# jakovdev/SequenceAligner

Measured on AMD Instinct MI355X. Metric: pair-alignments/sec, higher is better.
Workload: dtype u16x2; 1 GPU; cfg2: 10000 protein seqs x U[80,120], nw blosum62 {'gap_pen': 4}, all-vs-all packed triangular; pairs=49995000, cells=501594494441, parallelism=pair-range x1

## Files before the change

### sequencealigner_amd/csrc/sa_context.hip

```cpp
#include <algorithm>
#include <cmath>
#include <cstdio>
#include <cstdlib>
#include <cstring>

#include "sa_ctx.h"

bool sa_device_ready(int device)
{
	int count = 0;
	hipError_t err = hipGetDeviceCount(&count);
	if (err != hipSuccess || count <= 0) {
		sa_set_error("No HIP devices available (%s); libseqalign_hip has no CPU fallback",
			     err == hipSuccess ? "device count is 0" : hipGetErrorString(err));
		return false;
	}
	if (device < 0 || device >= count) {
		sa_set_error("HIP device %d out of range (%d visible)", device, count);
		return false;
	}
	SA_HIP_CHECK(hipSetDevice(device), return false);
	return true;
}

// ... 90 lines not shown
	in.min_len = ctx->min_len;
	in.method = ctx->sc.method;
	in.gap_ext = ctx->sc.gap_ext;
	in.sys_ok = ctx->sys_ok;
	in.pk_kmax = ctx->pk_kmax;
	in.pk16_kmax = ctx->pk16_kmax;
	in.pk16_f16_kmax = ctx->pk16_f16_kmax;
	in.pk_chunk_cap = ctx->pk_chunk_cap;
	in.pk_q = ctx->pk_q;
	in.pk_floor = ctx->pk_floor;
	in.pk_gain = ctx->pk_gain;
	in.pk_slack = ctx->pk_slack;
	in.persistent_wgs = ctx->persistent_wgs;
	in.env_chunk = ctx->env.chunk;
	in.no_sort = ctx->env.no_sort;
	return in;
}

namespace {
struct CtxDeleter {
	void operator()(sa_ctx *c) const { sa_ctx_destroy(c); }
};
}

static sa_ctx *ctx_create_impl(int device, struct sa_input in, const struct sa_scoring *sc)
{
	if (!sc) {
		sa_set_error("sa_ctx_create: null scoring");
		return nullptr;
	}
// ... 271 lines not shown
```

### sequencealigner_amd/csrc/sa_env.cpp

```cpp
#include "sa_env.h"

#include <algorithm>
#include <cstdlib>

static bool flag(const char *name) { return getenv(name) != nullptr; }
static int number(const char *name, int fallback, int lo, int hi)
{
	const char *v = getenv(name);
	if (!v || !*v)
		return fallback;
	return std::max(lo, std::min(hi, atoi(v)));
}

SaEnv sa_env_read()
{
	SaEnv e;
	e.force_generic = flag("SA_HIP_FORCE_GENERIC");
	e.no_pk = flag("SA_HIP_NO_PK");
	e.no_pk16 = flag("SA_HIP_NO_PK16");
	e.no_sort = flag("SA_HIP_NO_SORT");
	e.chunk = number("SA_HIP_CHUNK", 0, 1, 32);
	e.stagger = number("SA_HIP_STAGGER", 0, 0, 64);
	e.no_pin = flag("SA_HIP_NO_PIN");
	e.no_direct = flag("SA_HIP_NO_DIRECT");
	e.no_shells = flag("SA_HIP_NO_SHELLS");
	e.devices = number("SA_HIP_DEVICES", 0, 0, 1024);
	e.split = number("SA_HIP_SPLIT", 0, 0, 1024);
	e.gather = getenv("SA_HIP_GATHER") ? (atoi(getenv("SA_HIP_GATHER")) != 0) : -1;
	e.tiles_split = number("SA_HIP_TILES_SPLIT", 0, 0, 64);
	e.trace_batch_bytes = getenv("SA_HIP_TRACE_BATCH_BYTES") ? std::max(0LL, atoll(getenv("SA_HIP_TRACE_BATCH_BYTES"))) : 0LL;
	e.verbose = flag("SA_HIP_VERBOSE");
	e.stamps = flag("SA_HIP_STAMPS");
	e.stamps_dump = getenv("SA_HIP_STAMPS_DUMP");
	e.ztrace = flag("SA_HIP_ZTRACE");
	return e;
// ... 2 lines not shown
```

### sequencealigner_amd/csrc/sa_env.h

```cpp
#ifndef SA_ENV_H
#define SA_ENV_H

struct SaEnv {
	bool force_generic = false;
	bool no_pk = false;
	bool no_pk16 = false;
	bool no_sort = false;
	int chunk = 0;
	int stagger = 0;
	bool no_pin = false;
	bool no_direct = false;
	bool no_shells = false;
	int devices = 0;
	int split = 0;
	int gather = -1;
	int tiles_split = 0;
	long long trace_batch_bytes = 0;
	bool verbose = false;
	bool stamps = false;
	const char *stamps_dump = nullptr;
	bool ztrace = false;
};

SaEnv sa_env_read();
// ... 3 lines not shown
```

### sequencealigner_amd/csrc/sa_internal.h

```cpp
#ifndef SA_INTERNAL_H
#define SA_INTERNAL_H

#include <hip/hip_runtime.h>
#include <cstdint>
#include <cstdarg>
#include <string>
#include <vector>


#include "sa_shapes.h"

#define SA_HIP_CHECK(call, onfail)                                                  \
	if (hipError_t err__ = (call); err__ != hipSuccess) {                       \
		sa_set_error("%s failed: %s", #call, hipGetErrorString(err__));      \
		onfail;                                                              \
	} else                                                                      \
		(void)0

struct SaSeqStore {
	const uint8_t *codes;
	const struct sa_meta *meta;
	int32_t num;
};

// ... 19 lines not shown
	int64_t start, end;
	int32_t *out;
	int32_t out16;
	int32_t pconst;
	int32_t q;
	int32_t gap_g, gap_o, gap_e;
	int32_t delta;
	int32_t chunk;
	int32_t *long_scratch;
	int64_t long_stride;
	int32_t pk_base;
	const SaArranged *lvp;
	int32_t npart;
	int32_t out_nt;
	int32_t pk_f16;
	const int32_t *tlist;
	const int64_t *dense_off;
	int32_t *host_out;
	int32_t nlocal;
	const SaPkClassArgs *pkc;
	const uint32_t *ulist;
	int32_t tile_pair;
	int32_t npkc;
	unsigned *counter;
	int32_t rotate_prio;
	int32_t stagger;
	int32_t stamp_u;
	unsigned long long *stamps;
};

// ... 29 lines not shown
```

### sequencealigner_amd/csrc/sa_launch.hip

```cpp
#include <algorithm>
#include <cstdio>
#include <cstring>

#include "sa_ctx.h"


static void plan_free_device(sa_ctx::Plan &pl)
{
	for (auto &c : pl.dc) {
		(void)hipFree(c.d_jlist);
		(void)hipFree(c.d_tprefix);
		(void)hipFree(c.d_tlist);
		(void)hipFree(c.d_doff);
	}
	(void)hipFree(pl.d_segs);
	for (auto &b : pl.db) {
		(void)hipFree(b.d_args);
		(void)hipFree(b.d_ulist);
	}
	pl.dc.clear();
	pl.db.clear();
	pl.d_segs = nullptr;
}

// ... 248 lines not shown
	if (!ctx->timing)
		return true;
	SA_HIP_CHECK(hipEventRecord(e1, s), return false);
	ctx->events.push_back(sa_ctx::Timed{ name, e0, e1, pairs, cells });
	return true;
}

static Launch pk_launch(const sa_ctx *ctx, const sa_ctx::Plan &pl, size_t bi, int rk, bool share, unsigned *counters, const SaSysArgs &common)
{
	const SaHostBundle &b = pl.h.bundles[bi];
	Launch L;
	L.is_pk = true;
	L.g = b.g;
	L.klo = b.klo;
	L.f16 = b.f16;
	L.lds = (unsigned)sa_pk_lds_bytes(ctx->sc.method, b.g, b.kmax);
	SaSysArgs &a = L.a = common;
	a.pconst = ctx->pk_pconst;
	a.q = ctx->sc.method == SA_METHOD_SW ? 0 : ctx->pk_q;
	a.out_nt = ctx->out_is_host && !share ? 1 : 0;
	a.pk_f16 = b.f16;
	a.chunk = pl.h.chunk_pk;
	a.stagger = ctx->env.stagger;
	a.rotate_prio = ctx->sc.method != SA_METHOD_NW;
	a.pkc = pl.db[bi].d_args;
	a.ulist = pl.db[bi].d_ulist + b.ufirst[(size_t)rk];
	a.npkc = (int32_t)b.cls.size();
	a.nlocal = L.ntiles = b.nlocal[(size_t)rk];
	a.counter = counters + 2 * (SA_PK_CLASS0 + (int)bi);
	L.pairs = b.pairs[(size_t)rk];
	L.cells = b.cells[(size_t)rk];
	L.nstamp = (size_t)L.ntiles;
	L.stamp_words = 7 * L.nstamp;
	L.wgs = (int)std::min<int64_t>(ctx->persistent_wgs / 32 * (ctx->leave_room ? 3 : 4), L.ntiles);
	int klo_seen = b.kmax;
	for (int ci : b.cls)
		klo_seen = std::min(klo_seen, sa_pk_decode(pl.h.classes[(size_t)ci].cls).k);
	snprintf(L.name, sizeof(L.name), "sa_k_systolic_pk_bundle<%s,%d,%d,%s>[K%d-%d]", METHOD_TAG[ctx->sc.method], b.g, b.klo,
		 b.f16 ? "true" : "false", klo_seen, b.kmax);
	return L;
}

static bool long_scratch_ready(sa_ctx *ctx)
{
	if (ctx->d_long_scratch)
		return true;
	ctx->long_stride = 2 * (16 * ((int64_t)ctx->max_len + 1) + 64);
	const int64_t budget_ints = ((int64_t)4 << 30) / 4;
	const int64_t wpb = SA_SYS_WPB(64, true);
	ctx->long_wgs = (int)std::max<int64_t>(16, std::min<int64_t>(ctx->persistent_wgs / 4, budget_ints / (ctx->long_stride * wpb)));
	SA_HIP_CHECK(hipMalloc(&ctx->d_long_scratch, sizeof(int32_t) * (size_t)(ctx->long_stride * ctx->long_wgs * wpb)), return false);
	return true;
}

// ... 331 lines not shown
```

### sequencealigner_amd/csrc/sa_plan.cpp

```cpp
#include "sa_plan.h"
#include "sa_guard.h"

#include <algorithm>
#include <cmath>
#include <cstdlib>

int32_t sa_column_of(int64_t p)
{
	int64_t j = (int64_t)((1.0 + std::sqrt(1.0 + 8.0 * (double)p)) * 0.5);
	while (j * (j - 1) / 2 > p)
		--j;
	while ((j + 1) * j / 2 <= p)
		++j;
	return (int32_t)j;
}

SaPairPlan::SaPairPlan(const sa_meta *m, int32_t n) : num(n), pairs((int64_t)n * (n - 1) / 2), meta(m)
{
	len_prefix.assign((size_t)n + 1, 0);
	cell_prefix.assign((size_t)n + 1, 0);
	for (int32_t k = 0; k < n; k++) {
		len_prefix[(size_t)k + 1] = len_prefix[(size_t)k] + m[k].len;
		cell_prefix[(size_t)k + 1] = cell_prefix[(size_t)k] + (int64_t)m[k].len * len_prefix[(size_t)k];
	}
// ... 37 lines not shown
}

bool sa_arranged_exists(int32_t num, const SaArrKey &key)
{
	const int64_t wave_rows = (int64_t)key.ng * key.ch;
	return key.block > 0 && wave_rows > 0 && key.block % (wave_rows * SA_PK_WPB) == 0 && key.block <= num;
}

int sa_pk_arranged_keys(const SaPlanInputs &in, int pk_g, int pk_k, int32_t chunk_pk, bool host_out, SaArrKey (&lv)[SA_PK_SORT_LEVELS])
{
	for (auto &x : lv)
		x = SaArrKey{};
	if (in.no_sort || chunk_pk <= 0)
		return 0;
	const int ng = 64 / pk_g;
	const int32_t rows = sa_pk_wpb(in.method, pk_g, pk_k) * ng * chunk_pk;
	int nl = 0;
	for (int l = 0; l < SA_PK_SORT_LEVELS; l++) {
		const int32_t block = SA_PK_SORT_ROWS >> l;
		if (host_out || rows >= SA_PK_ROWS_OWN_BLOCK || block <= rows || block % rows != 0)
			continue;
		const SaArrKey key{ ng, chunk_pk, block };
		if (sa_arranged_exists(in.num, key))
			lv[nl++] = key;
	}
	if (nl < SA_PK_SORT_LEVELS) {
		const SaArrKey key{ ng, chunk_pk, rows };
		if (sa_arranged_exists(in.num, key))
			lv[nl++] = key;
	}
	return nl;
// ... 54 lines not shown
	std::vector<std::vector<int32_t>> jl((size_t)SA_PLAN_NCLASSES), tp((size_t)SA_PLAN_NCLASSES);
	std::vector<int64_t> cpairs((size_t)SA_PLAN_NCLASSES, 0), ccells((size_t)SA_PLAN_NCLASSES, 0);
	std::vector<std::vector<std::pair<int32_t, int32_t>>> rows_of((size_t)SA_PLAN_NCLASSES);
	std::vector<int64_t> lenpre((size_t)num + 1, 0);
	for (int32_t k = 0; k < num; k++)
		lenpre[(size_t)k + 1] = lenpre[(size_t)k] + in.meta[k].len;
	{
		const int64_t want_tiles = (int64_t)in.persistent_wgs * 6;
		const int64_t mine = world > 1 ? count / world : count;
		int32_t chunk = SA_SYS_CHUNK;
		while (chunk > 8 && mine / (4 * chunk) < want_tiles)
			chunk >>= 1;
		if (in.env_chunk)
			chunk = in.env_chunk;
		plan.chunk = chunk;
		const int64_t want_pk = (int64_t)in.persistent_wgs * 5 / 8;
		int32_t cpk = SA_SYS_CHUNK;
		while (cpk > 4 && mine / ((int64_t)2 * SA_PK_WPB * 8 * cpk) < want_pk)
			cpk >>= 1;
		if (in.env_chunk)
			cpk = in.env_chunk;
		cpk = std::min(cpk, in.pk_chunk_cap);
		plan.chunk_pk = cpk;
		constexpr int TWO_SIZES_BELOW = 16, SMALL_TILE_DIV = 4, SMALL_PAIRS_FRAC = 5;
		const int64_t slots = (int64_t)in.persistent_wgs / 8;
		if (!in.env_chunk && mine / ((int64_t)2 * SA_PK_WPB * 8 * cpk) < (int64_t)TWO_SIZES_BELOW * slots) {
			int32_t big = SA_SYS_CHUNK;
			while (big > 16 && 2 * mine / ((int64_t)2 * SA_PK_WPB * 8 * big) < 5 * slots)
				big >>= 1;
			big = std::min(std::max(big, cpk), in.pk_chunk_cap);
			if (big >= 16) {
				plan.chunk_pk = big;
				plan.chunk_pk_small = std::max(4, big / SMALL_TILE_DIV);
				const int64_t jlo = sa_column_of(start), jhi = sa_column_of(end - 1) + 1;
				int64_t lo = jlo, hi = jhi;
				while (lo < hi) {
					const int64_t mid = (lo + hi) / 2;
					if (mid * (mid - 1) / 2 - start >= count / SMALL_PAIRS_FRAC)
						hi = mid;
					else
						lo = mid + 1;
				}
				plan.j_small = (int32_t)lo;
// ... 33 lines not shown
			sa_set_error("%s", TOO_LARGE);
			return false;
		}
		jl[(size_t)cls].push_back(j);
		tp[(size_t)cls].push_back(tp[(size_t)cls].back() + (int32_t)tiles);
		cpairs[(size_t)cls] += ib - ia;
		ccells[(size_t)cls] += (int64_t)n * (lenpre[(size_t)ib] - lenpre[(size_t)ia]);
	}
	std::vector<int32_t> nparts((size_t)SA_PLAN_NCLASSES, 0);
	std::vector<std::vector<int32_t>> part_rows((size_t)SA_PLAN_NCLASSES);
	for (int cls = SA_PK_CLASS0; cls < SA_PLAN_NCLASSES; cls++) {
		const auto &rw = rows_of[(size_t)cls];
		if (rw.empty())
			continue;
		const SaPkCls pc = sa_pk_decode(cls);
		const int64_t rows = (int64_t)sa_pk_wpb(in.method, pc.g, pc.k) * (64 / pc.g) * (pc.small ? plan.chunk_pk_small : plan.chunk_pk);
		tp[(size_t)cls].push_back(0);
		std::vector<std::pair<int32_t, int32_t>> parts;
		for (size_t c = 0; c < rw.size(); c += 2) {
			const auto &a = rw[c], &b = rw[c + 1 < rw.size() ? c + 1 : c];
			const int64_t span = std::max(a.second, b.second) - std::min(a.first, b.first);
			const int64_t tiles = span / rows;
			if ((int64_t)tp[(size_t)cls].back() + tiles + (int64_t)parts.size() + 1 > ((int64_t)1 << SA_PK_UTILE_BITS)) {
				sa_set_error("%s", TOO_LARGE);
				return false;
			}
			tp[(size_t)cls].push_back(tp[(size_t)cls].back() + (int32_t)tiles);
			if (span % rows)
				parts.emplace_back((int32_t)(span % rows), (int32_t)(c / 2));
		}
		std::stable_sort(parts.begin(), parts.end(), [](const auto &x, const auto &y) { return x.first > y.first; });
// ... 42 lines not shown
		for (size_t ci = 0; ci < plan.classes.size(); ci++) {
			auto &cl = plan.classes[ci];
			const int cls = cl.cls;
			const bool is_pk = cls >= SA_PK_CLASS0;
			const int pk_g = is_pk ? sa_pk_decode(cls).g : 8;
			const int G = is_pk ? pk_g : cls == SA_SYS_CLASS_LONG ? 64 : SA_SYS_CLASSES[cls].G;
			const int K = is_pk ? sa_pk_decode(cls).k : cls == SA_SYS_CLASS_LONG ? 16 : SA_SYS_CLASSES[cls].K;
			const int64_t weight = (int64_t)(K + 6) * (G / 8);
			const auto &J = cl.jlist;
			const auto &T = cl.tprefix;
			std::vector<Geo> tiles((size_t)cl.ntiles);
			if (is_pk) {
				SaArrKey lv[SA_PK_SORT_LEVELS];
				sa_pk_arranged_keys(in, pk_g, K, cl.chunk, share_host, lv);
				const int32_t lvrows[SA_PK_SORT_LEVELS] = { lv[0].block, lv[1].block, lv[2].block, lv[3].block };
				const int32_t rows = sa_pk_wpb(in.method, pk_g, K) * (64 / pk_g) * cl.chunk;
				const auto &rw = rows_of[(size_t)cls];
				const int32_t npairs = (cl.ncols + 1) / 2, nfull = T[(size_t)npairs];
				for (int32_t t = 0; t < cl.ntiles; t++) {
					int32_t lo;
					if (t < nfull)
						lo = (int32_t)(std::upper_bound(T.begin(), T.begin() + npairs + 1, t) - T.begin()) - 1;
					else
						lo = T[(size_t)(npairs + 1 + (t - nfull))];
					const size_t c0 = (size_t)2 * (size_t)lo, c1 = c0 + 1 < rw.size() ? c0 + 1 : c0;
					Geo &g = tiles[(size_t)t];
					g.dup = c1 == c0;
					g.j[0] = J[c0], g.j[1] = J[c1];
					g.ia[0] = rw[c0].first, g.ib[0] = rw[c0].second;
					g.ia[1] = rw[c1].first, g.ib[1] = rw[c1].second;
					const int32_t ra = std::min(g.ia[0], g.ia[1]), rb = std::max(g.ib[0], g.ib[1]);
// ... 102 lines not shown
		}
	}
	const int nranks = std::max(world, 1);
	std::vector<int> order;
	for (size_t ci = 0; ci < plan.classes.size(); ci++)
		if (plan.classes[ci].cls >= SA_PK_CLASS0)
			order.push_back((int)ci);
	std::sort(order.begin(), order.end(), [&](int x, int y) { return plan.classes[(size_t)x].cls > plan.classes[(size_t)y].cls; });
	std::stable_partition(order.begin(), order.end(), [&](int x) { return !sa_pk_decode(plan.classes[(size_t)x].cls).small; });
	for (int ci : order) {
		const auto &cl = plan.classes[(size_t)ci];
		const int g = sa_pk_decode(cl.cls).g;
		const int k = sa_pk_decode(cl.cls).k;
		const int klo = sa_pk_bundle_klo(g, k);
		const int f16 = g == 8 || k <= in.pk16_f16_kmax ? 1 : 0;
		SaHostBundle *b = nullptr;
		for (auto &x : plan.bundles)
			if (x.g == g && x.klo == klo && x.f16 == f16)
				b = &x;
		if (!b) {
			plan.bundles.emplace_back();
			b = &plan.bundles.back();
			b->g = g, b->klo = klo, b->f16 = f16, b->kmax = k;
		}
		b->kmax = std::max(b->kmax, k);
		b->cls.push_back(ci);
	}
	for (auto &b : plan.bundles) {
		b.args.resize(b.cls.size());
		for (size_t x = 0; x < b.cls.size(); x++) {
			const auto &cl = plan.classes[(size_t)b.cls[x]];
			const int k = sa_pk_decode(cl.cls).k;
			SaHostPkArgs &a = b.args[x];
			sa_pk_arranged_keys(in, b.g, k, cl.chunk, share_host, a.lv);
			a.cls_index = b.cls[x];
			a.chunk = cl.chunk;
			a.ncols = cl.ncols;
			a.npart = cl.npart;
// ... 7 lines not shown
		b.pairs.assign((size_t)nranks, 0);
		b.cells.assign((size_t)nranks, 0);
		struct Part {
			int64_t work;
			uint32_t code, pair;
		};
		std::vector<Part> parts;
		for (int r = 0; r < nranks; r++) {
			parts.clear();
			for (size_t x = 0; x < b.cls.size(); x++) {
				const auto &cl = plan.classes[(size_t)b.cls[x]];
				const int32_t nfull = cl.ntiles - cl.npart;
				const auto &T = cl.tprefix;
				const int32_t npairs = (cl.ncols + 1) / 2;
				const bool small = sa_pk_decode(cl.cls).small;
				const int64_t full_rows = (int64_t)sa_pk_wpb(in.method, b.g, sa_pk_decode(cl.cls).k) * (64 / b.g) * cl.chunk;
				int32_t pair_of_full = 0;
				for (int32_t t = 0; t < cl.ntiles; t++) {
					uint32_t pair;
					if (t < nfull) {
						while (pair_of_full + 1 < npairs && T[(size_t)pair_of_full + 1] <= t)
							pair_of_full++;
						pair = (uint32_t)pair_of_full;
					} else {
						pair = (uint32_t)T[(size_t)(npairs + 1 + (t - nfull))];
					}
					if (world >= 1 && cl.owner[(size_t)t] != r)
						continue;
					const uint32_t code = ((uint32_t)x << SA_PK_UTILE_BITS) | (uint32_t)t;
					if (t < nfull && !small) {
						ul.push_back(code);
// ... 63 lines not shown
```

### sequencealigner_amd/csrc/sa_plan.h

```cpp
#ifndef SA_PLAN_H
#define SA_PLAN_H

#include <cstdint>
#include <string>
#include <utility>
#include <vector>

#include "sa_shapes.h"

int32_t sa_column_of(int64_t p);
inline int64_t sa_tri(int64_t j) { return j * (j - 1) / 2; }

struct SaPairPlan {
	int32_t num = 0;
	int64_t pairs = 0;
	const sa_meta *meta = nullptr;
	std::vector<int64_t> len_prefix;
	std::vector<int64_t> cell_prefix;
	SaPairPlan(const sa_meta *m, int32_t n);
	int64_t cells_before(int64_t p) const;
};

struct SaArrKey {
	int ng = 0, ch = 0;
// ... 4 lines not shown
inline int sa_pk_live(int32_t min_len, int g) { return 1 + (g - 1) / ((min_len > 1 ? min_len : 1) + 1); }

struct SaPlanInputs {
	int32_t num = 0;
	const sa_meta *meta = nullptr;
	int32_t min_len = 1;
	int method = 0;
	int32_t gap_ext = 0;
	bool sys_ok = false;
	int pk_kmax = 0, pk16_kmax = 0, pk16_f16_kmax = 0, pk_chunk_cap = SA_SYS_CHUNK;
	int32_t pk_q = 0, pk_floor = 0;
	int64_t pk_gain = 0, pk_slack = 0;
	int persistent_wgs = 256 * 32;
	int env_chunk = 0;
	bool no_sort = false;
};

struct SaKernelLimits {
	bool sys_ok = false;
	int32_t sys_pconst = 0, sys_q = 0;
	int64_t sys_gain = 0, sys_slack = 0;
	int pk_kmax = 0, pk16_kmax = 0, pk16_f16_kmax = 0, pk_chunk_cap = SA_SYS_CHUNK;
	int32_t pk_pconst = 0, pk_q = 0, pk_floor = 0;
	int64_t pk_gain = 0, pk_slack = 0, pk_extra = 0;
};
SaKernelLimits sa_kernel_limits(const sa_scoring &sc, int32_t max_len, int32_t min_len, bool force_generic, bool no_pk, bool no_pk16);

int32_t sa_pk_delta(const SaPlanInputs &in, int g, int k);
int32_t sa_pk_base(const SaPlanInputs &in, int g, int k);

// ... 26 lines not shown
struct SaHostSeg {
	int64_t src, dst;
	int32_t count, pos0, ia, ib, flags;
	int map_kind;
	SaArrKey key;
};

struct SaHostPkArgs {
	int cls_index = 0;
	int32_t ncols = 0, npart = 0, k = 0, delta = 0, pk_base = 0, chunk = 0;
	SaArrKey lv[SA_PK_SORT_LEVELS];
};

struct SaHostBundle {
	int g = 8, klo = 1, f16 = 1, kmax = 1;
	std::vector<int> cls;
	std::vector<SaHostPkArgs> args;
	std::vector<uint32_t> ulist;
	std::vector<int64_t> ufirst;
	std::vector<int32_t> nlocal;
	std::vector<int64_t> pairs, cells;
};

struct SaGenericShare {
	int64_t start, count, doff;
};

struct SaHostPlan {
	int64_t start = -1, count = -1;
	int32_t chunk = SA_SYS_CHUNK;
// ... 17 lines not shown
```

### sequencealigner_amd/csrc/sa_shapes.h

```cpp
#ifndef SA_SHAPES_H
#define SA_SHAPES_H

#include <cstdint>

#include "../../include/seqalign_hip.h"

#if defined(__HIPCC__)
#define SA_HD __host__ __device__
#else
#define SA_HD
#endif

enum : int { SA_CODE_SEP = 24, SA_CODE_NOP = 25, SA_CODE_ROWS = 26 };

void sa_set_error(const char *fmt, ...) __attribute__((format(printf, 1, 2)));


#define SA_SYS_CHUNK 32
#define SA_SYS_WPB(G, LONG) ((G) >= 32 ? 4 : 1)
#define SA_SYS_CLASS_LIST(X) \
	X(0, 8, 1) X(1, 8, 2) X(2, 8, 3) X(3, 8, 4) \
	X(4, 8, 5) X(5, 8, 6) X(6, 8, 7) X(7, 8, 8) \
	X(8, 8, 9) X(9, 8, 10) X(10, 8, 11) X(11, 8, 12) \
	X(12, 8, 13) X(13, 8, 14) X(14, 8, 15) X(15, 8, 16) \
// ... 5 lines not shown
	X(36, 64, 13) X(37, 64, 14) X(38, 64, 15) X(39, 64, 16)
struct SaSysClass {
	int G, K;
};
static const SaSysClass SA_SYS_CLASSES[] = {
#define SA_SYS_ENTRY(IDX, G_, K_) { G_, K_ },
	SA_SYS_CLASS_LIST(SA_SYS_ENTRY)
#undef SA_SYS_ENTRY
};
enum : int { SA_SYS_NCLASSES = (int)(sizeof(SA_SYS_CLASSES) / sizeof(SA_SYS_CLASSES[0])),
	     SA_SYS_CLASS_LONG = SA_SYS_NCLASSES,
	     SA_SYS_LONG_W = 1024 };

#define SA_PK_WPB 4
#define SA_PK_K16_WIDE 45
SA_HD constexpr int sa_pk_wpb(int method, int g, int k)
{
	return (g == 16 && k >= SA_PK_K16_WIDE) || (method == SA_METHOD_NW && g == 8 && k >= 17) ? 2 * SA_PK_WPB : SA_PK_WPB;
}
#define SA_PK_F16_MAX 0x7bff
#define SA_PK_ROWS_OWN_BLOCK 1024
#define SA_PK_SORT_LEVELS 4
#define SA_PK_SORT_ROWS 2048
#define SA_PK_KMAX 24
#define SA_PK_K_LIST(X) \
	X(1) X(2) X(3) X(4) X(5) X(6) X(7) X(8) X(9) X(10) X(11) X(12) \
	X(13) X(14) X(15) X(16) X(17) X(18) X(19) X(20) X(21) X(22) X(23) X(24)
#define SA_PK_K16_MIN 13
#define SA_PK16_KMAX 64
#define SA_PK16_F16_KMAX 52
#define SA_PK_K16_LIST(X) \
	X(13) X(14) X(15) X(16) X(17) X(18) X(19) X(20) X(21) X(22) X(23) X(24) X(25) X(26) \
	X(27) X(28) X(29) X(30) X(31) X(32) X(33) X(34) X(35) X(36) X(37) X(38) X(39) X(40) \
// ... 11 lines not shown
	const int32_t *rowmap;
	const int32_t *posmap;
	int32_t rows;
};
struct SaPkClassArgs {
	const int32_t *jlist;
	const int32_t *tprefix;
	const int64_t *dense_off;
	int32_t ncols, npart, k;
	int32_t delta, pk_base;
	int32_t chunk;
	SaArranged lv[SA_PK_SORT_LEVELS];
};
#define SA_PK_UTILE_BITS 28
SA_HD constexpr int sa_pk_lds_fixed(int g, int wpb) { return 416 * wpb * (64 / g); }
SA_HD constexpr int sa_pk_lds_bytes(int method, int g, int k) { return sa_pk_lds_fixed(g, sa_pk_wpb(method, g, k)) + SA_CODE_ROWS * ((k + 3) / 4) * 256; }
inline int sa_pk_bundle_klo(int g, int k) { return g == 8 ? 1 + (k - 1) / SA_PK_BUNDLE * SA_PK_BUNDLE : SA_PK_K16_MIN + (k - SA_PK_K16_MIN) / SA_PK_BUNDLE * SA_PK_BUNDLE; }


#define SA_SHARE_PAD(rows) (((rows) + 7) & ~7)

SA_HD inline int sa_pk_pick_level(const int32_t *lvrows, int32_t ra, int32_t rb, int32_t i_begin, int32_t tile_rows)
{
	int pick = -1;
	if (ra % tile_rows != 0)
		return pick;
	for (int l = SA_PK_SORT_LEVELS - 1; l >= 0; l--) {
		const int32_t sr = lvrows[l];
		if (sr <= 0)
			continue;
		const int32_t blk0 = i_begin / sr * sr;
// ... 17 lines not shown
```

### sequencealigner_amd/csrc/sa_systolic_pk.inc

```
#include "sa_internal.h"
#include <atomic>
#include <type_traits>
#if !defined(SA_PK_G) || (SA_PK_G != 8 && SA_PK_G != 16)
#error "define SA_PK_G (8 or 16) before including sa_systolic_pk.inc"
#endif
#if SA_PK_G == 16 && !defined(SA_PK16_PART)
#error "define SA_PK16_PART (0: K = 13..44, 1: K = 45..64) before including sa_systolic_pk.inc with SA_PK_G 16"
#endif

#define SA_PK_STORE(nt, v, p)                          \
	do {                                           \
		if (nt) {                              \
			asm volatile("");  \
			__builtin_nontemporal_store((v), (p)); \
		} else                                 \
			*(p) = (v);                    \
	} while (0)

#ifndef SA_PK_OPAQUE_TOKEN
#define SA_PK_OPAQUE_TOKEN 1
#endif
#ifndef SA_PK_QUIET_BLOCKS
#define SA_PK_QUIET_BLOCKS 0
#endif

namespace {

extern __shared__ __attribute__((aligned(256))) uint8_t sa_pk_lds[];

constexpr int CH = SA_SYS_CHUNK;
typedef unsigned short u16x2 __attribute__((ext_vector_type(2)));

__device__ __forceinline__ uint32_t pkmax(uint32_t a, uint32_t b)
{
	return __builtin_bit_cast(uint32_t, __builtin_elementwise_max(__builtin_bit_cast(u16x2, a), __builtin_bit_cast(u16x2, b)));
}
// ... 18 lines not shown
	if (G == 8)
		return (uint32_t)__builtin_amdgcn_update_dpp((int)lead, (int)src, 0x112, 0xf, 0xf, false);
	return (uint32_t)__builtin_amdgcn_update_dpp((int)lead, (int)src, 0x111, 0xf, 0xf, false);
}

template <typename T> __device__ __forceinline__ T *uniform_ptr(T *p)
{
	const uint64_t v = reinterpret_cast<uint64_t>(p);
	const uint32_t lo = __builtin_amdgcn_readfirstlane((uint32_t)v), hi = __builtin_amdgcn_readfirstlane((uint32_t)(v >> 32));
	typedef __attribute__((address_space(1))) T *global_ptr;
	return (T *)reinterpret_cast<global_ptr>(((uint64_t)hi << 32) | lo);
}

__device__ __forceinline__ int32_t uload(const int32_t *p) { return __builtin_amdgcn_readfirstlane(*p); }

template <int METHOD, int G, int K, bool F16>
__device__ __forceinline__ void pk_tile(const SaSysArgs &A, const int32_t t_raw, const int32_t ntiles)
{
	static_assert(G == 8 || G == 16, "packed kernels: 8- or 16-lane groups");
	constexpr int NG = 64 / G, WPB = sa_pk_wpb(METHOD, G, K), NGW = NG * WPB;
	constexpr int W = G * K;
	constexpr int PARTS = (K + 3) / 4;
	constexpr int NSLOT = G;
	constexpr int COPIES = 16 / G;
	constexpr int PARTSTRIDE = COPIES * NSLOT * 16;
	static_assert(PARTSTRIDE == 256, "a part spans all 64 banks");
	constexpr int ROWSTRIDE = PARTS * PARTSTRIDE;
	constexpr int PROF_BYTES = SA_CODE_ROWS * ROWSTRIDE;
	constexpr int TSHIFT = (SA_CODE_ROWS - 1) * ROWSTRIDE < 65536 ? 0 : 8;
	constexpr uint32_t TUNIT = (uint32_t)ROWSTRIDE >> TSHIFT;
	static_assert((SA_CODE_ROWS - 1) * TUNIT < 65536, "the token of a profile row must fit u16");
	uint8_t *const s_prof = sa_pk_lds + sa_pk_lds_fixed(G, WPB);
	static_assert(PROF_BYTES + sa_pk_lds_fixed(G, WPB) == sa_pk_lds_bytes(METHOD, G, K), "host and kernel agree on the LDS of a class");
	constexpr int OUT_HALFS = 2 * NG * CH;
	static_assert(WPB * OUT_HALFS * 2 >= SA_SUB_DIM * SA_SUB_DIM, "the staged matrix must fit the score storage");
	int16_t *const s_out_all = reinterpret_cast<int16_t *>(sa_pk_lds);
	constexpr int RING = 64;
	constexpr int GSTRIDE = 2 * RING + 16;
	uint16_t *const s_ring_all = reinterpret_cast<uint16_t *>(sa_pk_lds + WPB * OUT_HALFS * 2);
	static_assert(WPB * OUT_HALFS * 2 + WPB * NG * GSTRIDE * 2 == sa_pk_lds_fixed(G, WPB), "LDS carve");
	static_assert(sa_pk_lds_fixed(G, WPB) % 256 == 0, "the profile starts on a 256-byte boundary: a part spans all 64 banks");

	int lane_id = threadIdx.x;
	asm volatile("" : "+v"(lane_id));
	const int lane = lane_id & 63;
	const int wv = __builtin_amdgcn_readfirstlane(lane_id >> 6);
	int16_t *s_out = s_out_all + wv * OUT_HALFS;
	uint16_t *s_ring = s_ring_all + wv * (NG * GSTRIDE);
// ... 161 lines not shown
	const uint32_t base2 = pk2((uint32_t)A.pk_base);
	const uint32_t delta2 = pk2((uint32_t)A.delta);
	const uint32_t q2 = pk2((uint32_t)-A.q);
	const uint32_t cmask2 = (pad[0] == 0 ? 0xffffu : 0u) | (pad[1] == 0 ? 0xffff0000u : 0u);
	uint32_t V[K], Y[K];
	uint32_t vl[2];
	uint32_t xout = 0;
	uint32_t vbase;
	uint32_t fl = 0;
	uint32_t flead = 0, xlead = 0;
	uint32_t best = 0, carry = 0;
	const uint32_t e2 = pk2((uint32_t)-A.gap_e);
	const uint32_t gqs2 = pk2((uint32_t)(A.gap_e - A.gap_o));
	int32_t frame = 0;
	int nsep = 0;
	const uint32_t inj0 = METHOD == SA_METHOD_NW ? base2 : base2 - 2 * q2;
	vl[0] = vl[1] = vbase = inj0;
	if (METHOD == SA_METHOD_SW) {
		const uint32_t o2 = pk2((uint32_t)-A.gap_o);
		const uint32_t top = base2 - o2 - (uint32_t)lig * e2;
		vl[0] = base2 - o2 - e2;
		vl[1] = top;
		xout = top - e2;
		xlead = base2 - o2;
		flead = base2;
		fl = base2 - (uint32_t)(lig + 1) * e2;
		best = base2 - (uint32_t)lig * e2;
#pragma unroll
		for (int q = 0; q < K; q++)
			V[q] = top, Y[q] = top;
// ... 91 lines not shown
					}
					frame++;
				}
				if (METHOD == SA_METHOD_GA && leader) {
					if ((gm >> (s + 2)) & 1u) {
						vl[(s + 1) & 1] = vbase;
						vcur = vbase + q2;
					} else if ((gm >> (s + 1)) & 1u) {
						vl[(s + 1) & 1] = vbase + (q2 & cmask2);
					} else if ((gm >> s) & 1u) {
						vcur = vbase;
					}
				}
				if (lig == G - 1 && tk_cur == SEPWORD) {
					const uint32_t v = METHOD == SA_METHOD_SW ? carry : V[K - 1];
					const int32_t rebase = (frame - nsep) * A.delta - A.pk_base +
							       (METHOD == SA_METHOD_SW ? ((blk << 4) + s - (G - 1)) * A.gap_e : 0);
					s_out[grp * CH + nsep] = (int16_t)((int32_t)(v & 0xffffu) + rebase);
					s_out[NG * CH + grp * CH + nsep] = (int16_t)((int32_t)(v >> 16) + rebase);
					nsep++;
				}
			}
			const uint32_t tk_far = rbase[s + 2];
			const uint32_t vprev = vl[(s + 1) & 1];
			const uint8_t *const row_next = lane_prof + (tk_nxt << TSHIFT);
			auto reload = [&](int q_done) {
				if ((q_done & 3) == 3 || q_done == K - 1) {
					P[q_done >> 2] = *reinterpret_cast<const uint4 *>(row_next + (q_done >> 2) * PARTSTRIDE);
					if ((K & 3) != 0 && (q_done >> 2) == PARTS - 1)
						asm volatile("" ::"v"(P[PARTS - 1].y), "v"(P[PARTS - 1].z), "v"(P[PARTS - 1].w));
				}
			};
			uint32_t dnw[K];
			if (METHOD == SA_METHOD_NW) {
				dnw[0] = vprev + comp(P[0], 0);
#pragma unroll
				for (int q = 1; q < K; q++)
					dnw[q] = V[q - 1] + comp(P[q >> 2], q & 3);
#pragma unroll
				for (int p = 0; p < PARTS; p++)
					P[p] = *reinterpret_cast<const uint4 *>(row_next + p * PARTSTRIDE);
				if ((K & 3) != 0)
					asm volatile("" ::"v"(P[PARTS - 1].y), "v"(P[PARTS - 1].z), "v"(P[PARTS - 1].w));
				__builtin_amdgcn_sched_barrier(0);
			}
			if (METHOD == SA_METHOD_SW)
				vcur += 2 * e2;
			const uint32_t vleft = vcur = shift_in<G>(vcur, V[K - 1]);
			if (METHOD == SA_METHOD_SW) {
// ... 38 lines not shown
						const uint32_t m = pkmax(t0, x);
						if (q + 1 < K) {
							const uint32_t y = pkmax(pkmax(V[q + 1], Y[q + 1]), fl);
							Y[q + 1] = y;
							t0 = pkmax(V[q] + comp(P[(q + 1) >> 2], (q + 1) & 3), y);
							reload(q + 1);
						}
						best = pkmax(best, m);
						V[q] = m - gqs2;
						x = pkmax(V[q], x) - e2;
					}
				}
				best += e2;
				xout = x;
			} else if (METHOD == SA_METHOD_NW) {
				if (F16) {
#pragma unroll
					for (int q = 0; q < K; q++)
						V[q] = pkmax3<true>(dnw[q], V[q], q ? V[q - 1] : vleft);
				} else {
					uint32_t tq[K];
					tq[0] = pkmax(dnw[0], V[0]);
					if constexpr (K > 1)
						tq[1] = pkmax(dnw[1], V[1]);
#pragma unroll
					for (int q = 0; q < K; q++) {
						V[q] = pkmax(tq[q], q ? V[q - 1] : vleft);
						if (q + 2 < K)
							tq[q + 2] = pkmax(dnw[q + 2], V[q + 2]);
					}
				}
// ... 192 lines not shown
				if (METHOD == SA_METHOD_NW)
					score = raw + (m + nh[h]) * A.gap_g;
				else if (METHOD == SA_METHOD_GA)
					score = raw - A.q + (m + nh[h]) * A.gap_e;
				else
					score = raw;
				if (p16)
					SA_PK_STORE(pnt, (int16_t)score, &reinterpret_cast<int16_t *>(pout)[tri[h] + i - A.start]);
				else
					SA_PK_STORE(pnt, score, &pout[tri[h] + i - A.start]);
			}
		}
	}
}

template <int METHOD, int G, int KLO, bool F16>
__global__ __launch_bounds__(64 * sa_pk_wpb(METHOD, G, KLO)) void sa_k_systolic_pk_bundle(SaSysArgs A0)
{
	__shared__ int32_t s_next;
	constexpr int KMAX = G == 8 ? SA_PK_KMAX : SA_PK16_KMAX;
	if (A0.stagger > 0) {
		if (threadIdx.x == 0)
			s_next = (int32_t)(__builtin_amdgcn_s_getreg((3 << 11) | 4) & 3u);
		__syncthreads();
		const int32_t n = __builtin_amdgcn_readfirstlane(s_next) * A0.stagger;
		for (int32_t k = 0; k < n; k++)
			__builtin_amdgcn_s_sleep(127);
		__syncthreads();
	}
	const uint32_t wave_slot = __builtin_amdgcn_s_getreg((3 << 11) | 4);
	for (;;) {
		if (threadIdx.x == 0)
// ... 14 lines not shown
		A.dense_off = uniform_ptr(P.dense_off);
		A.ncols = __builtin_amdgcn_readfirstlane(P.ncols);
		A.npart = __builtin_amdgcn_readfirstlane(P.npart);
		A.delta = __builtin_amdgcn_readfirstlane(P.delta);
		A.pk_base = __builtin_amdgcn_readfirstlane(P.pk_base);
		A.rotate_prio = A0.rotate_prio ? (int32_t)(4u + (wave_slot & 3u)) : 0;
		A.chunk = __builtin_amdgcn_readfirstlane(P.chunk);
		A.lvp = P.lv;
		const int32_t ntiles = __builtin_amdgcn_readfirstlane(A.tprefix[(A.ncols + 1) >> 1]) + A.npart;
		const unsigned long long st0 = A0.stamps ? __builtin_amdgcn_s_memrealtime() : 0ull;
		const unsigned long long sc0 = A0.stamps ? __builtin_amdgcn_s_memtime() : 0ull;
		A.stamp_u = u;
		switch (__builtin_amdgcn_readfirstlane(P.k) - KLO) {
#define SA_BCASE(D)                                                  \
	case D:                                                      \
		if constexpr (KLO + D <= KMAX)                       \
			pk_tile<METHOD, G, KLO + D, F16>(A, t, ntiles); \
		break;
			SA_BCASE(0) SA_BCASE(1) SA_BCASE(2) SA_BCASE(3) SA_BCASE(4) SA_BCASE(5) SA_BCASE(6) SA_BCASE(7)
#undef SA_BCASE
		default:
			break;
		}
		if (A0.stamps && threadIdx.x == 0) {
			A0.stamps[3 * (size_t)u + 0] = st0;
			A0.stamps[3 * (size_t)u + 1] = __builtin_amdgcn_s_memrealtime();
			A0.stamps[3 * (size_t)u + 2] = sc0;
			A0.stamps[6 * (size_t)A0.nlocal + (size_t)u] = __builtin_amdgcn_s_memtime();
		}
	}
	if (threadIdx.x == 0) {
		__threadfence();
		if (atomicAdd(A0.counter + 1, 1u) == gridDim.x - 1) {
			atomicExch(A0.counter, 0u);
			atomicExch(A0.counter + 1, 0u);
		}
	}
}

template <int METHOD, int G, int KLO, bool F16>
hipError_t launch_bundle(const SaSysArgs &a, int wgs, unsigned lds_bytes, hipStream_t s)
{
	auto *kern = &sa_k_systolic_pk_bundle<METHOD, G, KLO, F16>;
	if (lds_bytes > 64 * 1024) {
		static std::atomic<unsigned long long> raised{ 0 };
		int dev = 0;
		(void)hipGetDevice(&dev);
		const unsigned long long bit = 1ull << (dev & 63);
		if (!(raised.load() & bit)) {
			(void)hipFuncSetAttribute(reinterpret_cast<const void *>(kern), hipFuncAttributeMaxDynamicSharedMemorySize,
						  sa_pk_lds_bytes(METHOD, G, KLO + SA_PK_BUNDLE - 1 < (G == 8 ? SA_PK_KMAX : SA_PK16_KMAX) ? KLO + SA_PK_BUNDLE - 1
														   : (G == 8 ? SA_PK_KMAX : SA_PK16_KMAX)));
			(void)hipGetLastError();
			raised.fetch_or(bit);
		}
	}
	static_assert(sa_pk_wpb(METHOD, G, KLO) == sa_pk_wpb(METHOD, G, KLO + SA_PK_BUNDLE - 1), "a bundle does not straddle the workgroup sizes");
	hipLaunchKernelGGL(kern, dim3(wgs), dim3(64 * sa_pk_wpb(METHOD, G, KLO)), lds_bytes, s, a);
	return hipGetLastError();
}

template <int METHOD> hipError_t launch_pk(int g, int klo, int f16, const SaSysArgs &a, int wgs, unsigned lds_bytes, hipStream_t s)
{
	if (g != SA_PK_G || !a.pkc || a.npkc < 1 || a.npkc > 2 * SA_PK_BUNDLE)
		return hipErrorInvalidValue;
#if SA_PK_G == 8
	if (!f16)
		return hipErrorInvalidValue;
	switch (klo) {
	case 1:
		return launch_bundle<METHOD, 8, 1, true>(a, wgs, lds_bytes, s);
	case 9:
		return launch_bundle<METHOD, 8, 9, true>(a, wgs, lds_bytes, s);
	case 17:
		return launch_bundle<METHOD, 8, 17, true>(a, wgs, lds_bytes, s);
	default:
		return hipErrorInvalidValue;
	}
#else
#define SA_B16(KLO_)                                                                        \
	case KLO_:                                                                          \
		return f16 ? launch_bundle<METHOD, 16, KLO_, true>(a, wgs, lds_bytes, s)    \
			   : launch_bundle<METHOD, 16, KLO_, false>(a, wgs, lds_bytes, s);
	switch (klo) {
#if SA_PK16_PART == 0
		SA_B16(13) SA_B16(21) SA_B16(29) SA_B16(37)
#else
// ... 34 lines not shown
```

Measured before the change: 3.436 billion pair-alignments/s.

## Add wide 8-wave workgroup shape for NW 8-lane classes K9-16

For NW with 8-lane groups and K in 9..16 (proteins of length 80-120 land here), the packed kernel now launches a separate 'wide' variant with twice the waves per workgroup, a waves_per_eu(6,6) hint, just-in-time diagonal computation instead of a precomputed dnw array to cut register pressure, and a slimmer separator-output path. The planner detects when most pairs fall in these classes and rescales chunk sizing and persistent workgroup counts (3 per CU slot instead of 4). The intent is better latency hiding and occupancy. The cost is more LDS per workgroup and coarser tiles, and SA_HIP_PK_NARROW restores the old shape.

```diff
diff --git a/sequencealigner_amd/csrc/sa_context.hip b/sequencealigner_amd/csrc/sa_context.hip
--- a/sequencealigner_amd/csrc/sa_context.hip
+++ b/sequencealigner_amd/csrc/sa_context.hip
@@ -128,6 +128,7 @@
 	in.persistent_wgs = ctx->persistent_wgs;
 	in.env_chunk = ctx->env.chunk;
 	in.no_sort = ctx->env.no_sort;
+	in.pk_narrow = ctx->env.pk_narrow;
 	return in;
 }
 
diff --git a/sequencealigner_amd/csrc/sa_env.cpp b/sequencealigner_amd/csrc/sa_env.cpp
--- a/sequencealigner_amd/csrc/sa_env.cpp
+++ b/sequencealigner_amd/csrc/sa_env.cpp
@@ -19,6 +19,7 @@
 	e.no_pk = flag("SA_HIP_NO_PK");
 	e.no_pk16 = flag("SA_HIP_NO_PK16");
 	e.no_sort = flag("SA_HIP_NO_SORT");
+	e.pk_narrow = flag("SA_HIP_PK_NARROW");
 	e.chunk = number("SA_HIP_CHUNK", 0, 1, 32);
 	e.stagger = number("SA_HIP_STAGGER", 0, 0, 64);
 	e.no_pin = flag("SA_HIP_NO_PIN");
diff --git a/sequencealigner_amd/csrc/sa_env.h b/sequencealigner_amd/csrc/sa_env.h
--- a/sequencealigner_amd/csrc/sa_env.h
+++ b/sequencealigner_amd/csrc/sa_env.h
@@ -6,6 +6,7 @@
 	bool no_pk = false;
 	bool no_pk16 = false;
 	bool no_sort = false;
+	bool pk_narrow = false;
 	int chunk = 0;
 	int stagger = 0;
 	bool no_pin = false;
diff --git a/sequencealigner_amd/csrc/sa_internal.h b/sequencealigner_amd/csrc/sa_internal.h
--- a/sequencealigner_amd/csrc/sa_internal.h
+++ b/sequencealigner_amd/csrc/sa_internal.h
@@ -57,6 +57,7 @@
 	int32_t npart;
 	int32_t out_nt;
 	int32_t pk_f16;
+	int32_t pk_wpb;
 	const int32_t *tlist;
 	const int64_t *dense_off;
 	int32_t *host_out;
diff --git a/sequencealigner_amd/csrc/sa_launch.hip b/sequencealigner_amd/csrc/sa_launch.hip
--- a/sequencealigner_amd/csrc/sa_launch.hip
+++ b/sequencealigner_amd/csrc/sa_launch.hip
@@ -286,12 +286,13 @@
 	L.g = b.g;
 	L.klo = b.klo;
 	L.f16 = b.f16;
-	L.lds = (unsigned)sa_pk_lds_bytes(ctx->sc.method, b.g, b.kmax);
+	L.lds = (unsigned)(sa_pk_lds_fixed(b.g, b.wpb) + sa_pk_prof_bytes(b.kmax));
 	SaSysArgs &a = L.a = common;
 	a.pconst = ctx->pk_pconst;
 	a.q = ctx->sc.method == SA_METHOD_SW ? 0 : ctx->pk_q;
 	a.out_nt = ctx->out_is_host && !share ? 1 : 0;
 	a.pk_f16 = b.f16;
+	a.pk_wpb = b.wpb;
 	a.chunk = pl.h.chunk_pk;
 	a.stagger = ctx->env.stagger;
 	a.rotate_prio = ctx->sc.method != SA_METHOD_NW;
@@ -304,12 +305,14 @@
 	L.cells = b.cells[(size_t)rk];
 	L.nstamp = (size_t)L.ntiles;
 	L.stamp_words = 7 * L.nstamp;
-	L.wgs = (int)std::min<int64_t>(ctx->persistent_wgs / 32 * (ctx->leave_room ? 3 : 4), L.ntiles);
+	const bool wide9 = b.wpb == 2 * SA_PK_WPB && sa_pk_two_shapes(ctx->sc.method, b.g, b.klo);
+	const int per_cu = wide9 ? (ctx->leave_room ? 2 : 3) : (ctx->leave_room ? 3 : 4);
+	L.wgs = (int)std::min<int64_t>(ctx->persistent_wgs / 32 * per_cu, L.ntiles);
 	int klo_seen = b.kmax;
 	for (int ci : b.cls)
 		klo_seen = std::min(klo_seen, sa_pk_decode(pl.h.classes[(size_t)ci].cls).k);
-	snprintf(L.name, sizeof(L.name), "sa_k_systolic_pk_bundle<%s,%d,%d,%s>[K%d-%d]", METHOD_TAG[ctx->sc.method], b.g, b.klo,
-		 b.f16 ? "true" : "false", klo_seen, b.kmax);
+	snprintf(L.name, sizeof(L.name), "sa_k_systolic_pk_bundle%s<%s,%d,%d,%s>[K%d-%d]", wide9 ? "_wide" : "", METHOD_TAG[ctx->sc.method], b.g,
+		 b.klo, b.f16 ? "true" : "false", klo_seen, b.kmax);
 	return L;
 }
 
diff --git a/sequencealigner_amd/csrc/sa_plan.cpp b/sequencealigner_amd/csrc/sa_plan.cpp
--- a/sequencealigner_amd/csrc/sa_plan.cpp
+++ b/sequencealigner_amd/csrc/sa_plan.cpp
@@ -75,7 +75,7 @@
 	if (in.no_sort || chunk_pk <= 0)
 		return 0;
 	const int ng = 64 / pk_g;
-	const int32_t rows = sa_pk_wpb(in.method, pk_g, pk_k) * ng * chunk_pk;
+	const int32_t rows = sa_pk_wpb(in.method, pk_g, pk_k, in.pk_narrow) * ng * chunk_pk;
 	int nl = 0;
 	for (int l = 0; l < SA_PK_SORT_LEVELS; l++) {
 		const int32_t block = SA_PK_SORT_ROWS >> l;
@@ -160,19 +160,28 @@
 		if (in.env_chunk)
 			chunk = in.env_chunk;
 		plan.chunk = chunk;
-		const int64_t want_pk = (int64_t)in.persistent_wgs * 5 / 8;
+		int64_t wide_pairs = 0;
+		if (!in.pk_narrow)
+			for (int32_t j = sa_column_of(start), j_end = sa_column_of(start + count - 1); j <= j_end; j++) {
+				const int k8 = (in.meta[j].len + 7) / 8;
+				if (k8 <= in.pk_kmax && sa_pk_two_shapes(in.method, 8, k8))
+					wide_pairs += std::min<int64_t>(j, start + count - sa_tri(j)) - std::max<int64_t>(0, start - sa_tri(j));
+			}
+		const bool wide = 2 * wide_pairs > count;
+		const int64_t tile_streams = wide ? 2 * SA_PK_WPB * 8 : SA_PK_WPB * 8;
+		const int64_t slots = (int64_t)in.persistent_wgs / 32 * (wide ? 3 : 4);
+		const int64_t want_pk = 5 * slots;
 		int32_t cpk = SA_SYS_CHUNK;
-		while (cpk > 4 && mine / ((int64_t)2 * SA_PK_WPB * 8 * cpk) < want_pk)
+		while (cpk > 4 && mine / (2 * tile_streams * cpk) < want_pk)
 			cpk >>= 1;
 		if (in.env_chunk)
 			cpk = in.env_chunk;
 		cpk = std::min(cpk, in.pk_chunk_cap);
 		plan.chunk_pk = cpk;
 		constexpr int TWO_SIZES_BELOW = 16, SMALL_TILE_DIV = 4, SMALL_PAIRS_FRAC = 5;
-		const int64_t slots = (int64_t)in.persistent_wgs / 8;
-		if (!in.env_chunk && mine / ((int64_t)2 * SA_PK_WPB * 8 * cpk) < (int64_t)TWO_SIZES_BELOW * slots) {
+		if (!in.env_chunk && mine / (2 * tile_streams * cpk) < (int64_t)TWO_SIZES_BELOW * slots) {
 			int32_t big = SA_SYS_CHUNK;
-			while (big > 16 && 2 * mine / ((int64_t)2 * SA_PK_WPB * 8 * big) < 5 * slots)
+			while (big > 16 && 2 * mine / (2 * tile_streams * big) < 5 * slots)
 				big >>= 1;
 			big = std::min(std::max(big, cpk), in.pk_chunk_cap);
 			if (big >= 16) {
@@ -236,7 +245,7 @@
 		if (rw.empty())
 			continue;
 		const SaPkCls pc = sa_pk_decode(cls);
-		const int64_t rows = (int64_t)sa_pk_wpb(in.method, pc.g, pc.k) * (64 / pc.g) * (pc.small ? plan.chunk_pk_small : plan.chunk_pk);
+		const int64_t rows = (int64_t)sa_pk_wpb(in.method, pc.g, pc.k, in.pk_narrow) * (64 / pc.g) * (pc.small ? plan.chunk_pk_small : plan.chunk_pk);
 		tp[(size_t)cls].push_back(0);
 		std::vector<std::pair<int32_t, int32_t>> parts;
 		for (size_t c = 0; c < rw.size(); c += 2) {
@@ -309,7 +318,7 @@
 				SaArrKey lv[SA_PK_SORT_LEVELS];
 				sa_pk_arranged_keys(in, pk_g, K, cl.chunk, share_host, lv);
 				const int32_t lvrows[SA_PK_SORT_LEVELS] = { lv[0].block, lv[1].block, lv[2].block, lv[3].block };
-				const int32_t rows = sa_pk_wpb(in.method, pk_g, K) * (64 / pk_g) * cl.chunk;
+				const int32_t rows = sa_pk_wpb(in.method, pk_g, K, in.pk_narrow) * (64 / pk_g) * cl.chunk;
 				const auto &rw = rows_of[(size_t)cls];
 				const int32_t npairs = (cl.ncols + 1) / 2, nfull = T[(size_t)npairs];
 				for (int32_t t = 0; t < cl.ntiles; t++) {
@@ -442,14 +451,15 @@
 		const int k = sa_pk_decode(cl.cls).k;
 		const int klo = sa_pk_bundle_klo(g, k);
 		const int f16 = g == 8 || k <= in.pk16_f16_kmax ? 1 : 0;
+		const int wpb = sa_pk_wpb(in.method, g, k, in.pk_narrow);
 		SaHostBundle *b = nullptr;
 		for (auto &x : plan.bundles)
-			if (x.g == g && x.klo == klo && x.f16 == f16)
+			if (x.g == g && x.klo == klo && x.f16 == f16 && x.wpb == wpb)
 				b = &x;
 		if (!b) {
 			plan.bundles.emplace_back();
 			b = &plan.bundles.back();
-			b->g = g, b->klo = klo, b->f16 = f16, b->kmax = k;
+			b->g = g, b->klo = klo, b->f16 = f16, b->kmax = k, b->wpb = wpb;
 		}
 		b->kmax = std::max(b->kmax, k);
 		b->cls.push_back(ci);
@@ -487,7 +497,7 @@
 				const auto &T = cl.tprefix;
 				const int32_t npairs = (cl.ncols + 1) / 2;
 				const bool small = sa_pk_decode(cl.cls).small;
-				const int64_t full_rows = (int64_t)sa_pk_wpb(in.method, b.g, sa_pk_decode(cl.cls).k) * (64 / b.g) * cl.chunk;
+				const int64_t full_rows = (int64_t)b.wpb * (64 / b.g) * cl.chunk;
 				int32_t pair_of_full = 0;
 				for (int32_t t = 0; t < cl.ntiles; t++) {
 					uint32_t pair;
diff --git a/sequencealigner_amd/csrc/sa_plan.h b/sequencealigner_amd/csrc/sa_plan.h
--- a/sequencealigner_amd/csrc/sa_plan.h
+++ b/sequencealigner_amd/csrc/sa_plan.h
@@ -42,6 +42,7 @@
 	int persistent_wgs = 256 * 32;
 	int env_chunk = 0;
 	bool no_sort = false;
+	bool pk_narrow = false;
 };
 
 struct SaKernelLimits {
@@ -98,6 +99,7 @@
 
 struct SaHostBundle {
 	int g = 8, klo = 1, f16 = 1, kmax = 1;
+	int wpb = SA_PK_WPB;
 	std::vector<int> cls;
 	std::vector<SaHostPkArgs> args;
 	std::vector<uint32_t> ulist;
diff --git a/sequencealigner_amd/csrc/sa_shapes.h b/sequencealigner_amd/csrc/sa_shapes.h
--- a/sequencealigner_amd/csrc/sa_shapes.h
+++ b/sequencealigner_amd/csrc/sa_shapes.h
@@ -43,9 +43,19 @@
 
 #define SA_PK_WPB 4
 #define SA_PK_K16_WIDE 45
-SA_HD constexpr int sa_pk_wpb(int method, int g, int k)
+#define SA_PK_NW8_WIDE_KLO 9
+#ifndef SA_PK_NW8_WIDE_KHI
+#define SA_PK_NW8_WIDE_KHI 16
+#endif
+SA_HD constexpr bool sa_pk_two_shapes(int method, int g, int k)
 {
-	return (g == 16 && k >= SA_PK_K16_WIDE) || (method == SA_METHOD_NW && g == 8 && k >= 17) ? 2 * SA_PK_WPB : SA_PK_WPB;
+	return method == SA_METHOD_NW && g == 8 && k >= SA_PK_NW8_WIDE_KLO && k <= SA_PK_NW8_WIDE_KHI;
+}
+SA_HD constexpr int sa_pk_wpb(int method, int g, int k, bool narrow = false)
+{
+	return (g == 16 && k >= SA_PK_K16_WIDE) || (method == SA_METHOD_NW && g == 8 && k >= 17) || (!narrow && sa_pk_two_shapes(method, g, k))
+		       ? 2 * SA_PK_WPB
+		       : SA_PK_WPB;
 }
 #define SA_PK_F16_MAX 0x7bff
 #define SA_PK_ROWS_OWN_BLOCK 1024
@@ -87,7 +97,8 @@
 };
 #define SA_PK_UTILE_BITS 28
 SA_HD constexpr int sa_pk_lds_fixed(int g, int wpb) { return 416 * wpb * (64 / g); }
-SA_HD constexpr int sa_pk_lds_bytes(int method, int g, int k) { return sa_pk_lds_fixed(g, sa_pk_wpb(method, g, k)) + SA_CODE_ROWS * ((k + 3) / 4) * 256; }
+SA_HD constexpr int sa_pk_prof_bytes(int k) { return SA_CODE_ROWS * ((k + 3) / 4) * 256; }
+SA_HD constexpr int sa_pk_lds_bytes(int method, int g, int k, bool narrow = false) { return sa_pk_lds_fixed(g, sa_pk_wpb(method, g, k, narrow)) + sa_pk_prof_bytes(k); }
 inline int sa_pk_bundle_klo(int g, int k) { return g == 8 ? 1 + (k - 1) / SA_PK_BUNDLE * SA_PK_BUNDLE : SA_PK_K16_MIN + (k - SA_PK_K16_MIN) / SA_PK_BUNDLE * SA_PK_BUNDLE; }
 
 
diff --git a/sequencealigner_amd/csrc/sa_systolic_pk.inc b/sequencealigner_amd/csrc/sa_systolic_pk.inc
--- a/sequencealigner_amd/csrc/sa_systolic_pk.inc
+++ b/sequencealigner_amd/csrc/sa_systolic_pk.inc
@@ -20,6 +20,9 @@
 #ifndef SA_PK_OPAQUE_TOKEN
 #define SA_PK_OPAQUE_TOKEN 1
 #endif
+#ifndef SA_PK_WIDE_JIT
+#define SA_PK_WIDE_JIT 1
+#endif
 #ifndef SA_PK_QUIET_BLOCKS
 #define SA_PK_QUIET_BLOCKS 0
 #endif
@@ -68,11 +71,12 @@
 
 __device__ __forceinline__ int32_t uload(const int32_t *p) { return __builtin_amdgcn_readfirstlane(*p); }
 
-template <int METHOD, int G, int K, bool F16>
+template <int METHOD, int G, int K, bool F16, int WPB>
 __device__ __forceinline__ void pk_tile(const SaSysArgs &A, const int32_t t_raw, const int32_t ntiles)
 {
 	static_assert(G == 8 || G == 16, "packed kernels: 8- or 16-lane groups");
-	constexpr int NG = 64 / G, WPB = sa_pk_wpb(METHOD, G, K), NGW = NG * WPB;
+	constexpr int NG = 64 / G, NGW = NG * WPB;
+	static_assert(WPB == sa_pk_wpb(METHOD, G, K, false) || WPB == sa_pk_wpb(METHOD, G, K, true), "a workgroup shape the host may plan for this class");
 	constexpr int W = G * K;
 	constexpr int PARTS = (K + 3) / 4;
 	constexpr int NSLOT = G;
@@ -85,7 +89,7 @@
 	constexpr uint32_t TUNIT = (uint32_t)ROWSTRIDE >> TSHIFT;
 	static_assert((SA_CODE_ROWS - 1) * TUNIT < 65536, "the token of a profile row must fit u16");
 	uint8_t *const s_prof = sa_pk_lds + sa_pk_lds_fixed(G, WPB);
-	static_assert(PROF_BYTES + sa_pk_lds_fixed(G, WPB) == sa_pk_lds_bytes(METHOD, G, K), "host and kernel agree on the LDS of a class");
+	static_assert(PROF_BYTES == sa_pk_prof_bytes(K), "host and kernel agree on the LDS of a class");
 	constexpr int OUT_HALFS = 2 * NG * CH;
 	static_assert(WPB * OUT_HALFS * 2 >= SA_SUB_DIM * SA_SUB_DIM, "the staged matrix must fit the score storage");
 	int16_t *const s_out_all = reinterpret_cast<int16_t *>(sa_pk_lds);
@@ -277,6 +281,8 @@
 	const uint32_t gqs2 = pk2((uint32_t)(A.gap_e - A.gap_o));
 	int32_t frame = 0;
 	int nsep = 0;
+	constexpr bool SLIM = WPB == 2 * SA_PK_WPB && sa_pk_two_shapes(METHOD, G, K);
+	int16_t *cap = s_out + grp * CH;
 	const uint32_t inj0 = METHOD == SA_METHOD_NW ? base2 : base2 - 2 * q2;
 	vl[0] = vl[1] = vbase = inj0;
 	if (METHOD == SA_METHOD_SW) {
@@ -398,11 +404,15 @@
 				}
 				if (lig == G - 1 && tk_cur == SEPWORD) {
 					const uint32_t v = METHOD == SA_METHOD_SW ? carry : V[K - 1];
-					const int32_t rebase = (frame - nsep) * A.delta - A.pk_base +
+					const int32_t rebase = (SLIM ? frame : frame - nsep) * A.delta - A.pk_base +
 							       (METHOD == SA_METHOD_SW ? ((blk << 4) + s - (G - 1)) * A.gap_e : 0);
-					s_out[grp * CH + nsep] = (int16_t)((int32_t)(v & 0xffffu) + rebase);
-					s_out[NG * CH + grp * CH + nsep] = (int16_t)((int32_t)(v >> 16) + rebase);
-					nsep++;
+					int16_t *const at = SLIM ? cap : s_out + grp * CH + nsep;
+					at[0] = (int16_t)((int32_t)(v & 0xffffu) + rebase);
+					at[NG * CH] = (int16_t)((int32_t)(v >> 16) + rebase);
+					if (SLIM)
+						cap++, frame--;
+					else
+						nsep++;
 				}
 			}
 			const uint32_t tk_far = rbase[s + 2];
@@ -415,8 +425,9 @@
 						asm volatile("" ::"v"(P[PARTS - 1].y), "v"(P[PARTS - 1].z), "v"(P[PARTS - 1].w));
 				}
 			};
-			uint32_t dnw[K];
-			if (METHOD == SA_METHOD_NW) {
+			constexpr bool NW_JIT = METHOD == SA_METHOD_NW && SA_PK_WIDE_JIT && WPB == 2 * SA_PK_WPB && sa_pk_two_shapes(METHOD, G, K);
+			[[maybe_unused]] uint32_t dnw[K];
+			if (METHOD == SA_METHOD_NW && !NW_JIT) {
 				dnw[0] = vprev + comp(P[0], 0);
 #pragma unroll
 				for (int q = 1; q < K; q++)
@@ -485,7 +496,21 @@
 				best += e2;
 				xout = x;
 			} else if (METHOD == SA_METHOD_NW) {
-				if (F16) {
+				if (NW_JIT) {
+					uint32_t d = vprev + comp(P[0], 0);
+#pragma unroll
+					for (int q = 0; q < K; q++) {
+						uint32_t dn = 0;
+						if (q + 1 < K) {
+							dn = V[q] + comp(P[(q + 1) >> 2], (q + 1) & 3);
+							reload(q + 1);
+						} else if (K == 1) {
+							reload(0);
+						}
+						V[q] = pkmax3<F16>(d, V[q], q ? V[q - 1] : vleft);
+						d = dn;
+					}
+				} else if (F16) {
 #pragma unroll
 					for (int q = 0; q < K; q++)
 						V[q] = pkmax3<true>(dnw[q], V[q], q ? V[q - 1] : vleft);
@@ -708,8 +733,13 @@
 	}
 }
 
-template <int METHOD, int G, int KLO, bool F16>
-__global__ __launch_bounds__(64 * sa_pk_wpb(METHOD, G, KLO)) void sa_k_systolic_pk_bundle(SaSysArgs A0)
+constexpr bool pk_shape_has(int method, int g, int k, int wpb)
+{
+	return wpb == sa_pk_wpb(method, g, k, true) || (wpb == 2 * SA_PK_WPB && sa_pk_two_shapes(method, g, k));
+}
+
+template <int METHOD, int G, int KLO, bool F16, int WPB>
+__device__ __forceinline__ void pk_bundle(const SaSysArgs &A0)
 {
 	__shared__ int32_t s_next;
 	constexpr int KMAX = G == 8 ? SA_PK_KMAX : SA_PK16_KMAX;
@@ -754,8 +784,8 @@
 		switch (__builtin_amdgcn_readfirstlane(P.k) - KLO) {
 #define SA_BCASE(D)                                                  \
 	case D:                                                      \
-		if constexpr (KLO + D <= KMAX)                       \
-			pk_tile<METHOD, G, KLO + D, F16>(A, t, ntiles); \
+		if constexpr (KLO + D <= KMAX && pk_shape_has(METHOD, G, KLO + D, WPB)) \
+			pk_tile<METHOD, G, KLO + D, F16, WPB>(A, t, ntiles); \
 		break;
 			SA_BCASE(0) SA_BCASE(1) SA_BCASE(2) SA_BCASE(3) SA_BCASE(4) SA_BCASE(5) SA_BCASE(6) SA_BCASE(7)
 #undef SA_BCASE
@@ -779,9 +809,28 @@
 }
 
 template <int METHOD, int G, int KLO, bool F16>
+__global__ __launch_bounds__(64 * sa_pk_wpb(METHOD, G, KLO, true)) void sa_k_systolic_pk_bundle(SaSysArgs A0)
+{
+	pk_bundle<METHOD, G, KLO, F16, sa_pk_wpb(METHOD, G, KLO, true)>(A0);
+}
+
+template <int METHOD, int G, int KLO, bool F16>
+__global__ __launch_bounds__(64 * 2 * SA_PK_WPB) __attribute__((amdgpu_waves_per_eu(6, 6))) void sa_k_systolic_pk_bundle_wide(SaSysArgs A0)
+{
+	static_assert(sa_pk_two_shapes(METHOD, G, KLO), "only the classes that have a second shape");
+	pk_bundle<METHOD, G, KLO, F16, 2 * SA_PK_WPB>(A0);
+}
+
+template <int METHOD, int G, int KLO, bool F16, bool WIDE = false>
 hipError_t launch_bundle(const SaSysArgs &a, int wgs, unsigned lds_bytes, hipStream_t s)
 {
-	auto *kern = &sa_k_systolic_pk_bundle<METHOD, G, KLO, F16>;
+	auto *kern = [] {
+		if constexpr (WIDE)
+			return &sa_k_systolic_pk_bundle_wide<METHOD, G, KLO, F16>;
+		else
+			return &sa_k_systolic_pk_bundle<METHOD, G, KLO, F16>;
+	}();
+	constexpr int WPB = WIDE ? 2 * SA_PK_WPB : sa_pk_wpb(METHOD, G, KLO, true);
 	if (lds_bytes > 64 * 1024) {
 		static std::atomic<unsigned long long> raised{ 0 };
 		int dev = 0;
@@ -795,8 +844,8 @@
 			raised.fetch_or(bit);
 		}
 	}
-	static_assert(sa_pk_wpb(METHOD, G, KLO) == sa_pk_wpb(METHOD, G, KLO + SA_PK_BUNDLE - 1), "a bundle does not straddle the workgroup sizes");
-	hipLaunchKernelGGL(kern, dim3(wgs), dim3(64 * sa_pk_wpb(METHOD, G, KLO)), lds_bytes, s, a);
+	static_assert(sa_pk_wpb(METHOD, G, KLO, true) == sa_pk_wpb(METHOD, G, KLO + SA_PK_BUNDLE - 1, true), "a bundle does not straddle the workgroup sizes");
+	hipLaunchKernelGGL(kern, dim3(wgs), dim3(64 * WPB), lds_bytes, s, a);
 	return hipGetLastError();
 }
 
@@ -811,6 +860,9 @@
 	case 1:
 		return launch_bundle<METHOD, 8, 1, true>(a, wgs, lds_bytes, s);
 	case 9:
+		if constexpr (sa_pk_two_shapes(METHOD, 8, 9))
+			if (a.pk_wpb == 2 * SA_PK_WPB)
+				return launch_bundle<METHOD, 8, 9, true, true>(a, wgs, lds_bytes, s);
 		return launch_bundle<METHOD, 8, 9, true>(a, wgs, lds_bytes, s);
 	case 17:
 		return launch_bundle<METHOD, 8, 17, true>(a, wgs, lds_bytes, s);
```

Result: slower. 3.192 billion pair-alignments/s (-7.1%).
